# arkworks-rs/circom-compat

Measured on AMD Instinct MI355X. Metric: Groth16 constraints/sec (BN254), higher is better.
Workload: dtype int32x9 (29-bit limbs of 254-bit Montgomery integers); 1 GPU; synthetic squaring-chain R1CS, 2^22-2 constraints, BN254, full prove (witness map + 4 G1 MSM + 1 G2 MSM + finalize), trapdoor key minted on GPU; log2_domain=22, num_constraints=4194302, n_vars=4194304, parallelism=single-gpu

## Files before the change

### circom_compat_amd/csrc/api.hip

```cpp
#include "../../include/g16_amd.h"

#include <stddef.h>
#include <stdlib.h>

#include <algorithm>
#include <mutex>

#include "ctx.h"

using namespace g16;

static_assert(offsetof(g16::ProofSums, B1) == sizeof(g16::G1XYZZ29) && offsetof(g16::ProofSums, L) == 2 * sizeof(g16::G1XYZZ29),
              "ProofSums must keep A, B1, L adjacent (batched reduction writes them as an array)");
static_assert(G16_PARTIAL_BYTES == g16::FIN_PARTIAL_BYTES, "partial record size out of sync");

namespace {
std::mutex g_err_mu;
std::string g_create_error;
}


namespace {

g16_status fail(g16_ctx* ctx, g16_status code, const std::string& msg) {
  if (ctx) ctx->err = msg;
  else {
    std::lock_guard<std::mutex> g(g_err_mu);
    g_create_error = msg;
  }
  return code;
}

template <class Fn>
g16_status guarded(g16_ctx* ctx, Fn fn) {
  try {
    if (ctx) G16_HIP(hipSetDevice(ctx->device));
    return fn();
  } catch (const HipError& e) {
    return fail(ctx, G16_ERR_HIP, e.what());
  } catch (const std::bad_alloc&) {
    return fail(ctx, G16_ERR_INTERNAL, "host allocation failed");
  } catch (const std::exception& e) {
    const bool dom = std::string(e.what()).find("PolynomialDegreeTooLarge") != std::string::npos;
    return fail(ctx, dom ? G16_ERR_DOMAIN_TOO_LARGE : G16_ERR_INTERNAL, e.what());
  }
}

void shard(uint32_t len, int rank, int world, uint32_t* lo, uint32_t* hi) {
  *lo = (uint32_t)((uint64_t)len * rank / world);
  *hi = (uint32_t)((uint64_t)len * (rank + 1) / world);
}

int work1_batch(const MsmConfig& cw, uint32_t wr, bool sharded) {
  return (cw.nb() / wr < (1u << 18) || sharded) ? 3 : 2;
}

size_t msm_state_bytes(const MsmConfig& cw, const MsmConfig& ch, uint32_t lw, uint32_t l_cnt, uint32_t lh,
                       uint32_t wr, bool sharded, bool own_w, bool own_h, bool view_w) {
  size_t b = 0;
  if (view_w) b += MsmSort::view_bytes_for(lw, cw);
  if (own_w) b += (size_t)cw.Pn * ((size_t)lw * (64 * 2 + 128) + (size_t)l_cnt * 64);
  if (own_h) b += (size_t)ch.Pn * lh * 64;
  b += MsmSort::bytes_for(lw, cw) + MsmSort::bytes_for(lh, ch);
  const uint32_t nc_w = ceil_div(cw.B, msm_red_chunk(cw, 1, wr)) * cw.D;
  const uint32_t nc_h = ceil_div(ch.B, msm_red_chunk(ch)) * ch.D;
  const uint32_t slots_w = cw.nb() + cw.max_lanes(), slots_h = ch.nb() + ch.max_lanes();
  b += msm_work_bytes<Fq>(slots_w, nc_w, cw.D, work1_batch(cw, wr, sharded)) + msm_work_bytes<Fq2>(slots_w, nc_w, cw.D, 1) +
       msm_work_bytes<Fq>(slots_h, nc_h, ch.D, 1);
  return b;
}

void plan_msm_configs(const g16_options& o, uint32_t lw, uint32_t l_cnt, uint32_t lh, uint32_t wr, bool sharded,
                      bool own_w, bool own_h, bool view_w, MsmConfig* cw, MsmConfig* ch) {
  if (own_w) *cw = msm_make_config(lw ? lw : 1, o.window_bits, o.planes);
  if (own_h) *ch = msm_make_config(lh ? lh : 1, o.window_bits, o.planes);
  if (o.planes > 0) return;
  size_t fr = 0, tot = 0;
  if (hipMemGetInfo(&fr, &tot) != hipSuccess) return;
  const size_t margin = std::min(((size_t)2 << 30) + fr / 50, fr / 4);
  const size_t budget = fr - margin;
  if (msm_state_bytes(*cw, *ch, lw, l_cnt, lh, wr, sharded, own_w, own_h, view_w) <= budget) return;
  auto layouts = [&](const MsmConfig& full, uint32_t len, bool own) {
    std::vector<MsmConfig> v{full};
    for (int pn = full.Pn - 1; own && pn >= 1; --pn) {
      const MsmConfig c = msm_make_config(len ? len : 1, o.window_bits, pn);
      if (c.Pn != v.back().Pn) v.push_back(c);
    }
    return v;
  };
  const std::vector<MsmConfig> vw = layouts(*cw, lw, own_w), vh = layouts(*ch, lh, own_h);
  long best = -1;
  size_t best_bytes = 0;
  for (const MsmConfig& a : vw)
    for (const MsmConfig& b : vh) {
      const size_t need = msm_state_bytes(a, b, lw, l_cnt, lh, wr, sharded, own_w, own_h, view_w);
      if (need > budget) continue;
      const long score = 5L * a.D + b.D;
      if (best < 0 || score < best || (score == best && need > best_bytes)) {
        best = score;
        best_bytes = need;
        *cw = a;
        *ch = b;
      }
    }
  if (best < 0) {
    if (!own_w && !own_h)
      throw std::runtime_error("the sort and partial-sum state of this ctx does not fit the device memory that is free (" +
                               std::to_string(fr >> 20) + " MiB)");
    throw std::runtime_error("the proving key does not fit this device's memory even with one plane per point (" +
                             std::to_string(fr >> 20) + " MiB free)");
  }
}

inline bool sched_r5() {
  static const bool v = [] { const char* e = getenv("G16_SCHED_R5"); return e && atoi(e) != 0; }();
  return v;
}

void collect_times(g16_ctx* c) {
  if (c->timer.enabled) c->timer.collect(c->st_ms, c->st_cnt);
}

struct BucketChunk {
  uint32_t count;
  const Fr* w;
  size_t w_stride;
  int32_t *abc, *spmv;
  U256* h;
  ProofSums* sums;
  MsmSort *sort_w, *sort_h, *sort_b;
  MsmWork<Fq> *work1, *workH;
  MsmWork<Fq2>* work2;
  Fr* rs;
  const uint8_t* rs_host;
  FinScratch* scr;
  uint8_t *rec, *proj;
  uint32_t rec_stride;
  uint8_t *rec_host, *proj_host;
  const MsmSort& sort_for_b(const g16_ctx* c) const { return c->sparse_b ? *sort_b : *sort_w; }
};

BucketChunk own_chunk(g16_ctx* c, const Fr* w_dev) {
  return BucketChunk{1,           w_dev,       c->N,        c->wm.abc.p, c->wm.spmv.partial.p, c->h_canon.p, c->sums_dev.p,
                     &c->sort_w,  &c->sort_h,  &c->sort_b,  &c->work1,   &c->workH,            &c->work2,
                     c->rs_dev.p, c->pin_io,   c->fin_scr.p, c->out_dev.p, c->part_dev(), (uint32_t)G16_PROOF_BYTES,
                     c->pin_io + 64, c->pin_io + 64 + G16_PROOF_BYTES};
}

void accumulate_ab(g16_ctx* c, const BucketChunk& ch, hipStream_t s, StageTimer* tm, bool fixup = true) {
  if (c->ptsA.stride == 2) {
    msm_accumulate_pair<Fq>(*ch.sort_w, c->ptsA, c->ptsB1, *ch.work1, 0, s, tm, fixup);
  } else {
    msm_accumulate<Fq>(*ch.sort_w, c->ptsA, 0, *ch.work1, 0, s, tm, fixup);
    msm_accumulate<Fq>(*ch.sort_w, c->ptsB1, 0, *ch.work1, 1, s, tm, fixup);
  }
}
void fixup_ab(g16_ctx* c, const BucketChunk& ch, hipStream_t q) {
  StageTimer* tm = c->timer.enabled ? &c->timer : nullptr;
  if (c->ptsA.stride == 2) {
    msm_fixup_pair<Fq>(*ch.sort_w, c->ptsA, c->ptsB1, *ch.work1, 0, q, tm);
  } else {
    msm_fixup<Fq>(*ch.sort_w, c->ptsA, 0, *ch.work1, 0, q, tm);
    msm_fixup<Fq>(*ch.sort_w, c->ptsB1, 0, *ch.work1, 1, q, tm);
  }
}

void enqueue_witness_sort(g16_ctx* c, const BucketChunk& ch) {
  hipStream_t s = c->stream;
  StageTimer* tm = c->timer.enabled ? &c->timer : nullptr;
  int id = tm ? tm->begin(ST_MSM_SORT, s) : -1;
  ch.sort_w->run(ch.w + 1 + c->w_lo, c->w_hi - c->w_lo, true, s, ch.count, ch.w_stride);
  if (tm) tm->end(id, s);
  if (c->sparse_b) {
    hipStream_t v = c->overlap ? c->red : s;
    G16_HIP(hipEventRecord(c->ev_view, s));
    G16_HIP(hipStreamWaitEvent(v, c->ev_view, 0));
    id = tm ? tm->begin(ST_MSM_SORT, v) : -1;
    ch.sort_b->run_view(*ch.sort_w, c->keep_b, v);
    if (tm) tm->end(id, v);
    G16_HIP(hipEventRecord(c->ev_view, v));
  }
}
void wait_for_b_view(g16_ctx* c, hipStream_t s) {
  if (c->sparse_b) G16_HIP(hipStreamWaitEvent(s, c->ev_view, 0));
}

template <class Hook, class Hook2>
void enqueue_witness_msms(g16_ctx* c, const BucketChunk& ch, Hook after_ab, Hook2 after_b2, bool sorted = false) {
  hipStream_t s = c->stream;
  StageTimer* tm = c->timer.enabled ? &c->timer : nullptr;
  ProofSums* S = ch.sums;
  const size_t ps = sizeof(ProofSums);
  if (!sorted) enqueue_witness_sort(c, ch);
  const uint32_t nb_eff = ch.count * c->cfg_w.nb() / (c->shard_buckets ? (uint32_t)c->world : 1u);
  const bool small = nb_eff < (1u << 18);
  const uint32_t b2_limit = c->world > 1 ? (1u << 18) : (1u << 16);
  const bool b2_off = c->overlap && nb_eff < b2_limit;
  const bool sharded = c->world > 1 || c->dist_wm;
  const bool mid = (nb_eff >= (1u << 15) && small) || (sharded && nb_eff >= (1u << 15));
  if (mid && c->overlap && ch.work1->batch >= 3) {
    hipStream_t q = c->red;
    accumulate_ab(c, ch, s, tm, false);
    G16_HIP(hipEventRecord(c->ev_acc[0], s));
    G16_HIP(hipStreamWaitEvent(q, c->ev_acc[0], 0));
    fixup_ab(c, ch, q);
    msm_reduce<Fq>(*ch.sort_w, *ch.work1, 0, 2, &S->A, q, tm, true, ps);
    after_ab(q);
    wait_for_b_view(c, s);
    msm_accumulate<Fq2>(ch.sort_for_b(c), c->ptsB2, 0, *ch.work2, 0, s, tm);
    G16_HIP(hipEventRecord(c->ev_acc[1], s));
    G16_HIP(hipStreamWaitEvent(q, c->ev_acc[1], 0));
    msm_reduce<Fq2>(ch.sort_for_b(c), *ch.work2, 0, 1, &S->B2, q, tm, true, ps);
    const bool r5 = sched_r5();
    hipStream_t ql = r5 ? q : c->side;
    if (!r5) after_b2();
    msm_accumulate<Fq>(*ch.sort_w, c->ptsL, c->l_idx_min, *ch.work1, 2, s, tm, false);
    G16_HIP(hipEventRecord(c->ev_acc[2], s));
    G16_HIP(hipStreamWaitEvent(ql, c->ev_acc[2], 0));
    msm_fixup<Fq>(*ch.sort_w, c->ptsL, c->l_idx_min, *ch.work1, 2, ql, tm);
    msm_reduce<Fq>(*ch.sort_w, *ch.work1, 2, 1, &S->L, ql, tm, true, ps);
    if (r5) after_b2();
    G16_HIP(hipEventRecord(c->ev_b2, q));
    G16_HIP(hipStreamWaitEvent(c->side, c->ev_b2, 0));
    G16_HIP(hipEventRecord(c->ev_side, c->side));
    return;
  }
  if (small && ch.work1->batch >= 3) {
    accumulate_ab(c, ch, s, tm);
    msm_accumulate<Fq>(*ch.sort_w, c->ptsL, c->l_idx_min, *ch.work1, 2, s, tm);
    msm_reduce<Fq>(*ch.sort_w, *ch.work1, 0, 3, &S->A, s, tm, false, ps);
    after_ab(s);
  } else {
    accumulate_ab(c, ch, s, tm);
    msm_reduce<Fq>(*ch.sort_w, *ch.work1, 0, 2, &S->A, s, tm, false, ps);
    after_ab(s);
    msm_run<Fq>(*ch.sort_w, c->ptsL, c->l_idx_min, *ch.work1, &S->L, s, tm, ps);
  }
  wait_for_b_view(c, s);
  msm_accumulate<Fq2>(ch.sort_for_b(c), c->ptsB2, 0, *ch.work2, 0, s, tm);
  hipStream_t rs = b2_off ? c->red : s;
  G16_HIP(hipEventRecord(c->ev_b2, s));
  G16_HIP(hipStreamWaitEvent(rs, c->ev_b2, 0));
  msm_reduce<Fq2>(ch.sort_for_b(c), *ch.work2, 0, 1, &S->B2, rs, tm, false, ps);
  G16_HIP(hipEventRecord(c->ev_b2, rs));
  if (rs != c->red) G16_HIP(hipStreamWaitEvent(c->red, c->ev_b2, 0));
  after_b2();
  G16_HIP(hipEventRecord(c->ev_b2, c->red));
  G16_HIP(hipStreamWaitEvent(c->side, c->ev_b2, 0));
  G16_HIP(hipEventRecord(c->ev_side, c->side));
}

void enqueue_h_msm(g16_ctx* c, const BucketChunk& ch) {
  hipStream_t s = c->stream;
  StageTimer* tm = c->timer.enabled ? &c->timer : nullptr;
  G16_HIP(hipStreamWaitEvent(s, c->ev_h, 0));
  msm_run<Fq>(*ch.sort_h, c->ptsH, 0, *ch.workH, &ch.sums->H, s, tm, sizeof(ProofSums));
}

template <class Hook, class Hook2>
void run_msms(g16_ctx* c, const BucketChunk& ch, Hook after_ab, Hook2 after_b2) {
  hipStream_t s = c->stream, x = c->overlap ? c->aux : c->stream;
  StageTimer* tm = c->timer.enabled ? &c->timer : nullptr;
  const uint32_t nb_eff = ch.count * c->cfg_w.nb() / (c->shard_buckets ? (uint32_t)c->world : 1u);
  const bool sort_first = !sched_r5() && c->overlap && c->world == 1 && nb_eff >= (1u << 18) && c->n <= (1u << 24);
  if (sort_first) enqueue_witness_sort(c, ch);
  G16_HIP(hipEventRecord(c->ev_w, s));
  G16_HIP(hipStreamWaitEvent(x, c->ev_w, 0));
  int id = tm ? tm->begin(ST_WITNESS_MAP, x) : -1;
  c->wm.run_batch(ch.w, ch.w_stride, ch.count, ch.abc, ch.spmv, ch.h, nullptr, x);
  if (tm) tm->end(id, x);
  id = tm ? tm->begin(ST_MSM_SORT, x) : -1;
  ch.sort_h->run(ch.h + c->h_lo, c->h_hi - c->h_lo, false, x, ch.count, c->wm.n);
  if (tm) tm->end(id, x);
  G16_HIP(hipEventRecord(c->ev_h, x));
  enqueue_witness_msms(c, ch, after_ab, after_b2, sort_first);
  enqueue_h_msm(c, ch);
}

template <class Hook>
void run_msms(g16_ctx* c, const BucketChunk& ch, Hook after_ab) {
  run_msms(c, ch, after_ab, [] {});
}

void begin_sharded(g16_ctx* c, const uint64_t r[4], const uint64_t s_[4]) {
  hipStream_t s = c->stream;
  memcpy(c->fixed_rs, r, 32);
  memcpy(c->fixed_rs + 4, s_, 32);
  G16_HIP(hipMemcpyAsync(c->rs_dev.p, c->fixed_rs, 64, hipMemcpyHostToDevice, s));
  G16_HIP(hipEventRecord(c->ev_start, s));
  G16_HIP(hipStreamWaitEvent(c->side, c->ev_start, 0));
  fin_fixed_dist(c->fin_tab.p, c->rs_dev.p, c->fin_scr.p, c->side);
  c->fixed_ready = true;
}

g16_status check_w(g16_ctx* c, size_t n_vars) {
  if (n_vars != c->N) return fail(c, G16_ERR_INVALID, "witness length != n_vars of the key");
  return G16_OK;
}

}

namespace g16 {

void rank_collect_times(g16_ctx* c) { collect_times(c); }

struct TabChunk {
  uint32_t count;
  const Fr* w;
  uint32_t w_stride;
  Fr* rs;
  const uint8_t* rs_host;
  int32_t *abc, *spmv;
  U256* h;
  ProofSums* sums;
  FinScratch* scr;
  G1XYZZ29 *part1, *partH;
  G2XYZZ29* part2;
  uint8_t *proj, *proj_host;
};

static void enqueue_prove_tables(g16_ctx* c, const TabChunk& ch) {
  hipStream_t s = c->stream;
  hipStream_t x = c->overlap ? c->red : s, q = c->overlap ? c->aux : s, sd = c->overlap ? c->side : s;
  StageTimer* tm = c->timer.enabled ? &c->timer : nullptr;
  const uint32_t n = ch.count;
  G16_HIP(hipMemcpyAsync(ch.rs, ch.rs_host, (size_t)64 * n, hipMemcpyHostToDevice, s));
  G16_HIP(hipEventRecord(c->ev_start, s));
  G16_HIP(hipStreamWaitEvent(q, c->ev_start, 0));
  int id = tm ? tm->begin(ST_MSM_TABLE_G2, q) : -1;
  c->tbl.run_g2_witness(ch.w + 1, ch.w_stride, ch.sums, ch.part2, n, q);
  if (tm) tm->end(id, q);
  G16_HIP(hipStreamWaitEvent(x, c->ev_start, 0));
  id = tm ? tm->begin(ST_WITNESS_MAP, x) : -1;
  c->wm.run_batch(ch.w, ch.w_stride, n, ch.abc, ch.spmv, ch.h, nullptr, x);
  if (tm) tm->end(id, x);
  id = tm ? tm->begin(ST_MSM_TABLE_G1, x) : -1;
  c->tbl.run_h(ch.h, c->wm.n, ch.sums, ch.partH, n, x);
  if (tm) tm->end(id, x);
  G16_HIP(hipEventRecord(c->ev_h, x));
  G16_HIP(hipStreamWaitEvent(sd, c->ev_start, 0));
  fin_fixed_dist(c->fin_tab.p, ch.rs, ch.scr, sd, n);
  fin_tab_pre(c->key_dev.p, ch.scr, sd, n);
  G16_HIP(hipEventRecord(c->ev_fixed, sd));
  G16_HIP(hipStreamWaitEvent(q, c->ev_fixed, 0));
  fin_tab_b(ch.sums, ch.scr, ch.proj, q, n);
  G16_HIP(hipEventRecord(c->ev_b2, q));
  id = tm ? tm->begin(ST_MSM_TABLE_G1, s) : -1;
  c->tbl.run_g1_witness(ch.w + 1, ch.w_stride, ch.rs, ch.sums, ch.part1, n, s);
  if (tm) tm->end(id, s);
  G16_HIP(hipStreamWaitEvent(s, c->ev_fixed, 0));
  id = tm ? tm->begin(ST_FINALIZE, s) : -1;
  fin_tab_ac(ch.sums, ch.scr, ch.proj, s, n);
  G16_HIP(hipStreamWaitEvent(s, c->ev_h, 0));
  fin_tab_c(ch.sums, ch.scr, ch.proj, s, n);
  if (tm) tm->end(id, s);
  G16_HIP(hipStreamWaitEvent(s, c->ev_b2, 0));
  G16_HIP(hipMemcpyAsync(ch.proj_host, ch.proj, (size_t)FIN_PROJ_BYTES * n, hipMemcpyDeviceToHost, s));
}

static void enqueue_prove_tables(g16_ctx* c, const Fr* w_dev) {
  const TabChunk ch{1,           w_dev,          c->N,          c->rs_dev.p,   c->pin_io,
                    c->wm.abc.p, c->wm.spmv.partial.p, c->h_canon.p, c->sums_dev.p, c->fin_scr.p,
                    c->tbl.part1.p, c->tbl.partH.p, c->tbl.part2.p, c->part_dev(), c->pin_io + 64 + G16_PROOF_BYTES};
  enqueue_prove_tables(c, ch);
}

static void proof_from_pin(g16_ctx* c, uint8_t* proof_out) {
  if (c->tbl.active) {
    fin_tab_host_affine(c->pin_io + 64 + G16_PROOF_BYTES, proof_out);
  } else {
    memcpy(proof_out, c->pin_io + 64, G16_PROOF_BYTES);
    fin_host_affine_c(c->pin_io + 64 + G16_PROOF_BYTES, proof_out);
  }
}

static void enqueue_prove_buckets(g16_ctx* c, const BucketChunk& ch) {
  hipStream_t s = c->stream;
  const uint32_t n = ch.count;
  G16_HIP(hipMemcpyAsync(ch.rs, ch.rs_host, (size_t)64 * n, hipMemcpyHostToDevice, s));
  G16_HIP(hipEventRecord(c->ev_start, s));
  G16_HIP(hipStreamWaitEvent(c->side, c->ev_start, 0));
  fin_fixed(c->fin_tab.p, ch.rs, ch.scr, c->side, n);
  G16_HIP(hipEventRecord(c->ev_fixed, c->side));
  run_msms(
      c, ch,
      [&](hipStream_t from) {
        G16_HIP(hipEventRecord(c->ev_ab, from));
        G16_HIP(hipStreamWaitEvent(c->side, c->ev_ab, 0));
        fin_var(c->key_dev.p, ch.sums, ch.rs, ch.scr, ch.rec, c->side, n, ch.rec_stride);
// ... 1172 lines not shown
```

### circom_compat_amd/csrc/field29.h

```cpp
#pragma once
#include "field.h"

#if defined(G16_EMU) && !defined(F29_NO_CHECK)
#include <assert.h>
#include <math.h>
#define F29_CHECK 1
#endif

namespace g16 {

namespace f29 {

constexpr int N = 9;
constexpr uint32_t MASK = (1u << 29) - 1u;

G16_HD int32_t opaque(int32_t x) {
#if defined(__HIP_DEVICE_COMPILE__) && !defined(F29_NO_OPAQUE)
  asm("" : "+v"(x));
#endif
  return x;
}

#if defined(F29_CHAIN_MAD) && defined(__HIP_DEVICE_COMPILE__)
__device__ __forceinline__ void mad_vv(int64_t& acc, int32_t a, int32_t b) {
// ... 361 lines not shown
    for (int k = 0; k < 2 * f29::N - 1; ++k) {
      __int128 s = 0;
      for (int i = 0; i < f29::N; ++i) {
        const int j = k - i;
        if (j < 0 || j >= f29::N) continue;
        __int128 x = (__int128)a.l[i] * b.l[j];
        __int128 y = (__int128)c.l[i] * d.l[j];
        s += (x < 0 ? -x : x) + (y < 0 ? -y : y);
      }
      s += (__int128)9 << 58;
      s += (__int128)1 << 36;
      assert(s < ((__int128)1 << 63) && "F29 mul2: column overflow");
    }
    long double v = fabsl(approx_over_p(a) * approx_over_p(b)) + fabsl(approx_over_p(c) * approx_over_p(d));
    assert(v < 168.9L && "F29 mul2: value bound exceeded");
  }
  static void check_mul_inputs(const F29& a, const F29& b) {
    {
      long double v = fabsl(approx_over_p(a) * approx_over_p(b));
      assert(v < 168.9L && "F29 mul: value bound exceeded");
    }
    for (int k = 0; k < 2 * f29::N - 1; ++k) {
      __int128 s = 0;
      for (int i = 0; i < f29::N; ++i) {
        const int j = k - i;
        if (j < 0 || j >= f29::N) continue;
        __int128 x = (__int128)a.l[i] * b.l[j];
        s += x < 0 ? -x : x;
      }
      s += (__int128)9 << 58;
      s += (__int128)1 << 36;
      assert(s < ((__int128)1 << 63) && "F29 mul: column overflow");
    }
  }
#endif
};

template <class P>
G16_HD F29<P> f29_inv(const F29<P>& a) {
  uint32_t e[8];
#pragma unroll
  for (int i = 0; i < 8; ++i) e[i] = P::MOD[i];
  e[0] -= 2;
  F29<P> r = F29<P>::one();
  bool started = false;
  for (int i = 7; i >= 0; --i) {
    for (int bit = 31; bit >= 0; --bit) {
      if (started) r = r.sqr();
      if ((e[i] >> bit) & 1) {
        r = r * a;
        started = true;
      }
    }
  }
  return r;
}

template <class P>
G16_HD F29<P> f29_inv_vartime(const F29<P>& a) {
  uint32_t u[8], v[8], x1[8], x2[8];
  a.canonical().pack(u);
  uint32_t nz = 0;
#pragma unroll
  for (int i = 0; i < 8; ++i) {
    nz |= u[i];
    v[i] = P::MOD[i];
    x1[i] = 0;
    x2[i] = 0;
  }
  if (!nz) return F29<P>::zero();
  x1[0] = 1;
  auto is_one = [](const uint32_t* t) {
    uint32_t o = t[0] ^ 1u;
    for (int i = 1; i < 8; ++i) o |= t[i];
    return o == 0;
  };
  auto shr1 = [](uint32_t* t, uint32_t top) {
    for (int i = 0; i < 7; ++i) t[i] = (t[i] >> 1) | (t[i + 1] << 31);
    t[7] = (t[7] >> 1) | (top << 31);
  };
  auto halve_mod = [&](uint32_t* x) {
    uint32_t top = 0;
    if (x[0] & 1u) {
      uint64_t c = 0;
      for (int i = 0; i < 8; ++i) {
        c += (uint64_t)x[i] + P::MOD[i];
        x[i] = (uint32_t)c;
        c >>= 32;
      }
      top = (uint32_t)c;
    }
    shr1(x, top);
  };
  auto geq = [](const uint32_t* s, const uint32_t* t) {
    for (int i = 7; i >= 0; --i)
      if (s[i] != t[i]) return s[i] > t[i];
    return true;
  };
  auto sub = [](uint32_t* s, const uint32_t* t) {
    uint64_t br = 0;
    for (int i = 0; i < 8; ++i) {
      const uint64_t d = (uint64_t)s[i] - t[i] - br;
      s[i] = (uint32_t)d;
      br = (d >> 32) & 1;
    }
    return (uint32_t)br;
  };
  auto sub_mod = [&](uint32_t* s, const uint32_t* t) {
    if (sub(s, t)) {
      uint64_t c = 0;
      for (int i = 0; i < 8; ++i) {
        c += (uint64_t)s[i] + P::MOD[i];
        s[i] = (uint32_t)c;
        c >>= 32;
      }
    }
  };
  for (int guard = 0; guard < 2048 && !is_one(u) && !is_one(v); ++guard) {
    while (!(u[0] & 1u)) {
      shr1(u, 0);
      halve_mod(x1);
    }
    while (!(v[0] & 1u)) {
      shr1(v, 0);
      halve_mod(x2);
    }
    if (geq(u, v)) {
      sub(u, v);
      sub_mod(x1, x2);
    } else {
      sub(v, u);
      sub_mod(x2, x1);
    }
  }
  const uint32_t(&res)[8] = is_one(u) ? x1 : x2;
  return F29<P>::unpack(res) * F29<P>::from_limbs(F29<P>::C::R3);
}

template <class P>
struct F29x2 {
  F29<P> c0, c1;
  using B = F29<P>;
  static G16_HD F29x2 zero() { return F29x2{B::zero(), B::zero()}; }
  static G16_HD F29x2 one() { return F29x2{B::one(), B::zero()}; }
  G16_HD bool limbs_all_zero() const { return c0.limbs_all_zero() && c1.limbs_all_zero(); }
  friend G16_HD F29x2 operator+(const F29x2& a, const F29x2& b) { return F29x2{a.c0 + b.c0, a.c1 + b.c1}; }
  friend G16_HD F29x2 operator-(const F29x2& a, const F29x2& b) { return F29x2{a.c0 - b.c0, a.c1 - b.c1}; }
  G16_HD F29x2 neg() const { return F29x2{c0.neg(), c1.neg()}; }
  G16_HD F29x2 dbl() const { return F29x2{c0.dbl(), c1.dbl()}; }
  G16_HD F29x2 carry() const { return F29x2{c0.carry(), c1.carry()}; }
  friend G16_HD F29x2 operator*(const F29x2& a, const F29x2& b) {
    return F29x2{B::mul_sub(a.c0, b.c0, a.c1, b.c1), B::mul2(a.c0, b.c1, a.c1, b.c0)};
  }
  G16_HD F29x2 sqr() const { return F29x2{B::mul_sub(c0, c0, c1, c1), c0.dbl() * c1}; }
  static G16_HD F29x2 mul_sub(const F29x2& a, const F29x2& b, const F29x2& c, const F29x2& d) {
    return (a * b - c * d).carry();
  }
  G16_HD bool is_zero_mod_p() const { return c0.is_zero_mod_p() && c1.is_zero_mod_p(); }
  G16_HD bool maybe_zero_mod_p() const { return c0.maybe_zero_mod_p() && c1.maybe_zero_mod_p(); }
  G16_HD F29x2 canonical() const { return F29x2{c0.canonical(), c1.canonical()}; }
  static G16_HD F29x2 from_mont256(const Fq2& a) {
    return F29x2{B::from_mont256(a.c0), B::from_mont256(a.c1)};
  }
  G16_HD Fq2 to_mont256() const { return Fq2{c0.to_mont256(), c1.to_mont256()}; }
};
template <class P>
G16_HD F29x2<P> f29_inv(const F29x2<P>& a) {
  F29<P> n = f29_inv(F29<P>::mul2(a.c0, a.c0, a.c1, a.c1));
  return F29x2<P>{a.c0 * n, (a.c1 * n).neg()};
}
template <class P>
G16_HD F29x2<P> f29_inv_vartime(const F29x2<P>& a) {
  F29<P> n = f29_inv_vartime(F29<P>::mul2(a.c0, a.c0, a.c1, a.c1));
  return F29x2<P>{a.c0 * n, (a.c1 * n).neg()};
}

using Fq29 = F29<FqParams>;
using Fq2x29 = F29x2<FqParams>;

template <class F> struct Lazy;
template <> struct Lazy<Fq> {
  using type = F29<FqParams>;
  static G16_HD type load_packed(const Fq& raw) { return type::unpack(raw.v); }
  static G16_HD Fq store_packed(const type& a) {
    Fq r;
    a.pack_internal(r.v);
    return r;
  }
};
template <> struct Lazy<Fq2> {
  using type = F29x2<FqParams>;
  static G16_HD type load_packed(const Fq2& raw) {
    return type{F29<FqParams>::unpack_opaque(raw.c0.v), F29<FqParams>::unpack_opaque(raw.c1.v)};
  }
  static G16_HD Fq2 store_packed(const type& a) {
    Fq2 r;
    a.c0.pack_internal(r.c0.v);
    a.c1.pack_internal(r.c1.v);
    return r;
  }
};

using Fr29 = F29<FrParams>;

}
```

### circom_compat_amd/csrc/msm.h

```cpp
#pragma once
#include <stdlib.h>
#include "common.h"
#include "ec29.h"

namespace g16 {

constexpr int MSM_ACC_THREADS = 128;
#ifdef G16_EMU
constexpr int MSM_ACC_BLOCKS = 48;
constexpr int MSM_ACC_BLOCKS_G2 = 32;
#else
constexpr int MSM_ACC_BLOCKS = 3072;
constexpr int MSM_ACC_BLOCKS_G2 = 2048;
#endif
constexpr int MSM_MIN_SEG = 8;
constexpr int MSM_SMALL_MULTI = 32;
constexpr int MSM_RED_CHUNK = 16;
constexpr uint32_t MSM_IDX_BITS_WIDE = 27, MSM_IDX_BITS_NARROW = 26;

struct MsmConfig {
  int c = 0;
  int W = 0;
  int Pn = 1;
  int D = 0;
  uint32_t B = 0;
  uint32_t idx_bits = MSM_IDX_BITS_NARROW;
  uint32_t max_points() const { return 1u << idx_bits; }
  uint32_t lanes = MSM_ACC_BLOCKS * MSM_ACC_THREADS;
  uint32_t lanes2 = MSM_ACC_BLOCKS_G2 * MSM_ACC_THREADS;
  uint32_t nb() const { return (uint32_t)D * B; }
  uint32_t max_lanes() const { return lanes > lanes2 ? lanes : lanes2; }
};

constexpr int MSM_PART_BITS_MAX = 12;
inline int msm_part_bits(uint32_t nb) {
  int bits = 10;
  while (bits < MSM_PART_BITS_MAX && (((uint64_t)nb + ((uint64_t)1 << bits) - 1) >> bits) > 4096u) ++bits;
  return bits;
}
inline int msm_part_shift(uint32_t nb) {
  int bits = 0;
  while (((uint64_t)1 << bits) < nb) ++bits;
  const int pb = msm_part_bits(nb);
  return bits > pb ? bits - pb : 0;
}

inline uint32_t msm_red_chunk(const MsmConfig& cfg, uint32_t nbatch = 1, uint32_t world = 1, bool hidden = false) {
  const uint64_t per_launch = (uint64_t)nbatch * cfg.D * cfg.B / (world ? world : 1);
  const uint32_t target = (hidden && per_launch <= (1u << 17)) ? 32768u : 65536u;
  uint32_t ch = (uint32_t)(((uint64_t)nbatch * cfg.D * cfg.B) / ((uint64_t)target * (world ? world : 1)));
  if (ch < 1) ch = 1;
  if (ch > (uint32_t)MSM_RED_CHUNK) ch = (uint32_t)MSM_RED_CHUNK;
  if (world > 1) {
    uint32_t p2 = 1;
    while (p2 * 2 <= ch) p2 *= 2;
    ch = p2;
    const uint32_t part = 1u << msm_part_shift(cfg.nb());
    if (ch > part) ch = part;
  }
  return ch;
}

MsmConfig msm_make_config(size_t len, int c_override, int planes_override);

struct alignas(8) MsmPair {
  uint32_t x;
  uint32_t y;
};

G16_HD uint32_t msm_seg_len(uint32_t M, uint32_t lanes) {
  uint32_t S = (uint32_t)(((uint64_t)M + lanes - 1) / lanes);
  return S < (uint32_t)MSM_MIN_SEG ? (uint32_t)MSM_MIN_SEG : S;
}

struct MsmSort {
  MsmConfig cfg;
  uint32_t cap = 0, len = 0;
  uint32_t nproof = 1, nproof_cap = 1;
  uint32_t nbt() const { return nproof * cfg.nb(); }
  DevBuf<MsmPair> part;
  DevBuf<uint32_t> count, offset, cursor, entries, multi_l, meta, multi_l2, meta2, scan_tmp;
  uint32_t lanes_of(bool g2) const { return g2 ? cfg.lanes2 : cfg.lanes; }
  const uint32_t* large_list(bool g2) const { return g2 ? multi_l2.p : multi_l.p; }
  const uint32_t* large_meta(bool g2) const { return g2 ? meta2.p : meta.p; }
  DevBuf<uint32_t> part_off;
  DevBuf<uint32_t> blk_hist, blk_off;
  int rank = 0, world = 1;
  DevBuf<uint32_t> range;
  const uint32_t* range_dev() const { return world > 1 ? range.p : nullptr; }

  void init(uint32_t capacity, const MsmConfig& cfg, uint32_t nproof_cap = 1);
  void set_shard(int rank, int world);
  void run(const void* scalars, uint32_t n, bool mont, hipStream_t stream, uint32_t nproof = 1, size_t stride = 0);
  void init_view(uint32_t capacity, const MsmConfig& cfg, uint32_t nproof_cap = 1);
  void release_view() {
    count.release(); offset.release(); cursor.release(); entries.release(); multi_l.release();
    meta.release(); multi_l2.release(); meta2.release(); scan_tmp.release();
    cap = len = 0;
  }
  void run_view(const MsmSort& src, const uint32_t* keep_bits, hipStream_t stream);
  static size_t view_bytes_for(uint32_t capacity, const MsmConfig& cfg, uint32_t nproof = 1) {
    const uint64_t M = (uint64_t)nproof * capacity * cfg.W;
    return (size_t)(M * 4 + 3 * ((uint64_t)nproof * cfg.nb() + 1) * 4 + 2 * (M / ((uint64_t)MSM_MIN_SEG * MSM_SMALL_MULTI) + 2) * 4 + 4096);
  }
  size_t device_bytes() const;
  static size_t bytes_for(uint32_t capacity, const MsmConfig& cfg, uint32_t nproof = 1);
};

template <class F>
using MsmAcc = XYZZ29<typename Lazy<F>::type>;

template <class F>
struct MsmPoints {
  MsmConfig cfg;
  uint32_t count = 0;
  DevBuf<Affine<F>> pts;
  const Affine<F>* view = nullptr;
  uint32_t stride = 1, off = 0;
  const Affine<F>* data() const { return view ? view : pts.p; }
  void init(const Affine<F>* host_points, uint32_t count, const MsmConfig& cfg, hipStream_t stream);
  static void init_pair(MsmPoints& a, MsmPoints& b, const Affine<F>* host_a, const Affine<F>* host_b,
                        uint32_t count, const MsmConfig& cfg, hipStream_t stream);
  void init_from_device(const Affine<F>* dev_points, uint32_t count, const MsmConfig& cfg,
                        hipStream_t stream);
};

#ifdef G16_EMU
constexpr uint32_t MSM_FIX_CAP = 512;
#else
constexpr uint32_t MSM_FIX_CAP = 2048;
#endif
struct MsmFixList {
  uint32_t count;
  uint32_t overflow;
  uint32_t slot[MSM_FIX_CAP];
  uint32_t entry[MSM_FIX_CAP];
};

template <class F>
struct MsmWork {
  int batch = 1;
  uint32_t slots = 0, ncontrib = 0;
  int sets = 1;
  DevBuf<MsmAcc<F>> partial;
  DevBuf<MsmAcc<F>> contrib;
  DevBuf<MsmAcc<F>> bsum;
  DevBuf<MsmAcc<F>> wsum;
  DevBuf<MsmFixList> fix;
  void init(uint32_t n_slots, uint32_t n_contrib, int max_sets, int batch = 1);
};

template <class F>
inline size_t msm_work_bytes(uint32_t n_slots, uint32_t n_contrib, int max_sets, int batch) {
  return (size_t)batch * ((size_t)n_slots + n_contrib + (size_t)257 * max_sets) * sizeof(MsmAcc<F>) +
         (size_t)batch * sizeof(MsmFixList);
}

template <class F>
void msm_run(const MsmSort& s, const MsmPoints<F>& pts, uint32_t idx_min, MsmWork<F>& work,
             MsmAcc<F>* out_dev, hipStream_t stream, StageTimer* tm = nullptr, size_t out_stride = 0);
template <class F>
void msm_accumulate(const MsmSort& s, const MsmPoints<F>& pts, uint32_t idx_min, MsmWork<F>& work,
                    int slot, hipStream_t stream, StageTimer* tm = nullptr, bool fixup = true);
template <class F>
void msm_fixup(const MsmSort& s, const MsmPoints<F>& pts, uint32_t idx_min, MsmWork<F>& work, int slot,
               hipStream_t stream, StageTimer* tm = nullptr);
template <class F>
void msm_accumulate_pair(const MsmSort& s, const MsmPoints<F>& a, const MsmPoints<F>& b,
                         MsmWork<F>& work, int slot, hipStream_t stream, StageTimer* tm = nullptr,
                         bool fixup = true);
template <class F>
void msm_fixup_pair(const MsmSort& s, const MsmPoints<F>& a, const MsmPoints<F>& b, MsmWork<F>& work,
                    int slot, hipStream_t stream, StageTimer* tm = nullptr);
template <class F>
void msm_reduce(const MsmSort& s, MsmWork<F>& work, int first_slot, int nbatch, MsmAcc<F>* out_dev,
                hipStream_t stream, StageTimer* tm = nullptr, bool hidden = false, size_t out_stride = 0);
inline uint32_t msm_contrib_cap(const MsmConfig& cfg, uint32_t nproof_cap) {
  uint32_t m = 1;
  for (uint32_t z = 1; z <= nproof_cap; ++z)
    for (uint32_t nbatch = 1; nbatch <= 3; ++nbatch)
      for (int hidden = 0; hidden < 2; ++hidden) {
        const uint32_t rc = msm_red_chunk(cfg, nbatch * z, 1, hidden != 0);
        const uint32_t v = (uint32_t)(((uint64_t)cfg.B + rc - 1) / rc) * (uint32_t)cfg.D * z;
        if (v > m) m = v;
      }
  return m;
}



}
```

### circom_compat_amd/csrc/msm_curve.inc.h

```cpp
#pragma once
#include <stdlib.h>

#include "msm.h"

namespace g16 {

namespace {

constexpr int ACC_THREADS = MSM_ACC_THREADS;
constexpr uint32_t MSM_EXACT_BLOCKS = 256;

inline bool acc_fast() {
  static const bool v = [] { const char* e = getenv("G16_ACC_FAST"); return !e || atoi(e) != 0; }();
  return v;
}
template <class F>
constexpr bool acc_is_g1() { return sizeof(F) == sizeof(Fq); }
constexpr int COMB_THREADS = 64;
constexpr int SUM_THREADS = 128;

template <class F>
__global__ void __launch_bounds__(128) k_precompute_planes(Affine<F>* pts, uint32_t count, int Pn,
                                                           int shift_bits, uint32_t stride,
                                                           uint32_t off) {
// ... 424 lines not shown
  b.off = 1;
  a.pts.alloc((size_t)2 * c.Pn * (n ? n : 1));
  a.view = nullptr;
  b.view = a.pts.p;
  if (!n) return;
  const size_t rec = sizeof(Affine<F>);
  G16_HIP(hipMemcpy2DAsync(a.pts.p, 2 * rec, host_a, rec, rec, n, hipMemcpyHostToDevice, stream));
  G16_HIP(hipMemcpy2DAsync(a.pts.p + 1, 2 * rec, host_b, rec, rec, n, hipMemcpyHostToDevice, stream));
  for (uint32_t h = 0; h < 2; ++h)
    G16_LAUNCH((k_precompute_planes<F>), ceil_div(n, 128), 128, 0, stream, a.pts.p, n, c.Pn,
               c.c * c.D, 2u, h);
}

template <class F>
void MsmWork<F>::init(uint32_t n_slots, uint32_t n_contrib, int max_sets, int batch_) {
  slots = n_slots ? n_slots : 1;
  ncontrib = n_contrib ? n_contrib : 1;
  sets = max_sets;
  batch = batch_;
  partial.alloc((size_t)batch * slots);
  contrib.alloc((size_t)batch * ncontrib);
  bsum.alloc((size_t)batch * 256 * sets);
  wsum.alloc((size_t)batch * sets);
  fix.alloc((size_t)batch);
  G16_HIP(hipMemset(fix.p, 0, (size_t)batch * sizeof(MsmFixList)));
}

template <class F>
void msm_accumulate(const MsmSort& s, const MsmPoints<F>& P, uint32_t idx_min, MsmWork<F>& work,
                    int slot, hipStream_t stream, StageTimer* tm, bool fixup) {
  const MsmConfig& cfg = s.cfg;
  const uint32_t nb = s.nbt();
  const int acc_stage = sizeof(F) == sizeof(Fq) ? ST_MSM_ACC_G1 : ST_MSM_ACC_G2;
  if (slot < 0 || slot >= work.batch) throw std::runtime_error("msm_accumulate: bad workspace slot");
  const uint32_t lanes = s.lanes_of(sizeof(F) != sizeof(Fq));
  const uint32_t grid = lanes / ACC_THREADS;
#ifdef G16_DEBUG_GATHER
  static const bool mask_set = [] {
    if (const char* e = getenv("G16_DEBUG_GATHER_MASK")) {
      const uint32_t m = (uint32_t)strtoul(e, nullptr, 0);
      G16_HIP(hipMemcpyToSymbol(HIP_SYMBOL(g_gather_mask), &m, sizeof m));
    }
    return true;
  }();
  (void)mask_set;
#endif
  int id = tm ? tm->begin(acc_stage, stream) : -1;
  MsmAcc<F>* out = work.partial.p + (size_t)slot * work.slots;
  const uint32_t* en = (const uint32_t*)s.entries.p;
  const uint32_t* of = (const uint32_t*)s.offset.p;
  if constexpr (acc_is_g1<F>()) {
    if (acc_fast()) {
      MsmFixList* fix = work.fix.p + slot;
      if (P.stride == 2)
        G16_LAUNCH((k_bucket_accumulate<F, 2, false, true>), grid, ACC_THREADS, 0, stream, P.data() + P.off,
                   P.count, idx_min, cfg.idx_bits, en, of, nb, lanes, out, (size_t)0, fix);
      else
        G16_LAUNCH((k_bucket_accumulate<F, 1, false, true>), grid, ACC_THREADS, 0, stream, P.data(), P.count,
                   idx_min, cfg.idx_bits, en, of, nb, lanes, out, (size_t)0, fix);
      if (tm) tm->end(id, stream);
      if (fixup) msm_fixup<F>(s, P, idx_min, work, slot, stream, tm);
      return;
    }
  }
  if (P.stride == 2)
    G16_LAUNCH((k_bucket_accumulate<F, 2, false, false>), grid, ACC_THREADS, 0, stream, P.data() + P.off,
               P.count, idx_min, cfg.idx_bits, en, of, nb, lanes, out, (size_t)0, (MsmFixList*)nullptr);
  else
    G16_LAUNCH((k_bucket_accumulate<F, 1, false, false>), grid, ACC_THREADS, 0, stream, P.data(), P.count,
               idx_min, cfg.idx_bits, en, of, nb, lanes, out, (size_t)0, (MsmFixList*)nullptr);
  if (tm) tm->end(id, stream);
}

template <class F>
void msm_fixup(const MsmSort& s, const MsmPoints<F>& P, uint32_t idx_min, MsmWork<F>& work, int slot,
               hipStream_t stream, StageTimer* tm) {
  if constexpr (!acc_is_g1<F>()) {
    return;
  } else {
  if (!acc_fast()) return;
  const int tid = tm ? tm->begin(ST_MSM_FIXUP, stream) : -1;
  const MsmConfig& cfg = s.cfg;
  const uint32_t nb = s.nbt();
  const uint32_t lanes = s.lanes_of(sizeof(F) != sizeof(Fq));
  const uint32_t grid = lanes / ACC_THREADS;
  MsmAcc<F>* out = work.partial.p + (size_t)slot * work.slots;
  const uint32_t* en = (const uint32_t*)s.entries.p;
  const uint32_t* of = (const uint32_t*)s.offset.p;
  MsmFixList* fix = work.fix.p + slot;
  const uint32_t grid_x = grid < MSM_EXACT_BLOCKS ? grid : MSM_EXACT_BLOCKS;
  if (P.stride == 2) {
    G16_LAUNCH((k_acc_fixup<F, 2>), 1, 256, 0, stream, P.data() + P.off, P.count, idx_min, cfg.idx_bits, fix, out, (size_t)0);
    G16_LAUNCH((k_bucket_accumulate<F, 2, false, false>), grid_x, ACC_THREADS, 0, stream, P.data() + P.off,
               P.count, idx_min, cfg.idx_bits, en, of, nb, lanes, out, (size_t)0, fix);
  } else {
    G16_LAUNCH((k_acc_fixup<F, 1>), 1, 256, 0, stream, P.data(), P.count, idx_min, cfg.idx_bits, fix, out, (size_t)0);
    G16_LAUNCH((k_bucket_accumulate<F, 1, false, false>), grid_x, ACC_THREADS, 0, stream, P.data(), P.count,
               idx_min, cfg.idx_bits, en, of, nb, lanes, out, (size_t)0, fix);
  }
  if (tm) tm->end(tid, stream);
  }
}

template <class F>
void msm_accumulate_pair(const MsmSort& s, const MsmPoints<F>& A, const MsmPoints<F>& B,
                         MsmWork<F>& work, int slot, hipStream_t stream, StageTimer* tm, bool fixup) {
  const MsmConfig& cfg = s.cfg;
  const uint32_t nb = s.nbt();
  const int acc_stage = ST_MSM_ACC_G1_PAIR;
  if (slot < 0 || slot + 2 > work.batch) throw std::runtime_error("msm_accumulate_pair: bad workspace slot");
  if (A.stride != 2 || B.stride != 2 || A.data() != B.data() || A.off != 0 || B.off != 1 ||
      A.count != B.count)
    throw std::runtime_error("msm_accumulate_pair: the queries are not an interleaved pair");
  const uint32_t grid = cfg.lanes / (ACC_THREADS / 2);
  int id = tm ? tm->begin(acc_stage, stream) : -1;
  const uint32_t* en = (const uint32_t*)s.entries.p;
  const uint32_t* of = (const uint32_t*)s.offset.p;
  MsmAcc<F>* out = work.partial.p + (size_t)slot * work.slots;
  if constexpr (sizeof(F) == sizeof(Fq)) {
    if (acc_fast()) {
      G16_LAUNCH((k_bucket_accumulate<F, 2, true, true>), grid, ACC_THREADS, 0, stream, A.data(), A.count, 0u,
                 cfg.idx_bits, en, of, nb, cfg.lanes, out, (size_t)work.slots, work.fix.p + slot);
      if (tm) tm->end(id, stream);
      if (fixup) msm_fixup_pair<F>(s, A, B, work, slot, stream, tm);
      return;
    }
  }
  G16_LAUNCH((k_bucket_accumulate<F, 2, true, false>), grid, ACC_THREADS, 0, stream, A.data(), A.count, 0u,
             cfg.idx_bits, en, of, nb, cfg.lanes, out, (size_t)work.slots, (MsmFixList*)nullptr);
  if (tm) tm->end(id, stream);
}

template <class F>
void msm_fixup_pair(const MsmSort& s, const MsmPoints<F>& A, const MsmPoints<F>& B, MsmWork<F>& work,
                    int slot, hipStream_t stream, StageTimer* tm) {
  (void)B;
  if constexpr (sizeof(F) == sizeof(Fq)) {
    if (!acc_fast()) return;
    const int tid = tm ? tm->begin(ST_MSM_FIXUP, stream) : -1;
    const MsmConfig& cfg = s.cfg;
    const uint32_t nb = s.nbt();
    const uint32_t grid = cfg.lanes / (ACC_THREADS / 2);
    MsmAcc<F>* out = work.partial.p + (size_t)slot * work.slots;
    MsmFixList* fix = work.fix.p + slot;
    const uint32_t grid_x = grid < MSM_EXACT_BLOCKS ? grid : MSM_EXACT_BLOCKS;
    G16_LAUNCH((k_acc_fixup<F, 2>), 1, 256, 0, stream, A.data(), A.count, 0u, cfg.idx_bits, fix, out, (size_t)work.slots);
    G16_LAUNCH((k_bucket_accumulate<F, 2, true, false>), grid_x, ACC_THREADS, 0, stream, A.data(), A.count, 0u,
               cfg.idx_bits, (const uint32_t*)s.entries.p, (const uint32_t*)s.offset.p, nb, cfg.lanes, out,
               (size_t)work.slots, fix);
    if (tm) tm->end(tid, stream);
  }
}

template <class F>
void msm_reduce(const MsmSort& s, MsmWork<F>& work, int first_slot, int nbatch, MsmAcc<F>* out_dev,
                hipStream_t stream, StageTimer* tm, bool hidden, size_t out_stride) {
  const MsmConfig& cfg = s.cfg;
  const uint32_t nb = s.nbt();
  const uint32_t sets = (uint32_t)cfg.D * s.nproof;
  if (first_slot < 0 || nbatch < 1 || first_slot + nbatch > work.batch)
    throw std::runtime_error("msm_reduce: bad workspace slots");
  MsmAcc<F>* partial = work.partial.p + (size_t)first_slot * work.slots;
  int id = tm ? tm->begin(ST_MSM_REDUCE, stream) : -1;
  const bool g2 = sizeof(F) != sizeof(Fq);
  const uint32_t lanes = s.lanes_of(g2);
  G16_LAUNCH((k_combine_large<F>), dim3(1024, nbatch), COMB_THREADS, COMB_THREADS * sizeof(MsmAcc<F>),
             stream, s.large_list(g2), s.large_meta(g2),
             (const uint32_t*)s.offset.p, nb, lanes, partial, (size_t)work.slots);
  const uint32_t* rng = s.range_dev();
  const uint32_t red_chunk = msm_red_chunk(cfg, (uint32_t)nbatch * s.nproof, (uint32_t)s.world, hidden);
  const uint32_t cps = ceil_div(cfg.B, red_chunk);
  const uint32_t nchunks = cps * sets;
  if (nchunks > work.ncontrib) throw std::runtime_error("msm_reduce: contribution buffer too small");
  if ((int)sets > work.sets) throw std::runtime_error("msm_reduce: more bucket sets than the workspace holds");
  MsmAcc<F>* contrib = work.contrib.p + (size_t)first_slot * work.ncontrib;
  MsmAcc<F>* bsum = work.bsum.p + (size_t)first_slot * 256 * work.sets;
  MsmAcc<F>* wsum = work.wsum.p + (size_t)first_slot * work.sets;
  G16_LAUNCH((k_bucket_reduce<F>), dim3(ceil_div(nchunks, 64), nbatch), 64, 0, stream,
             (const MsmAcc<F>*)partial, (const uint32_t*)s.offset.p, nb, lanes, cfg.B, red_chunk,
             cps, nchunks, contrib, (size_t)work.slots, rng);
  uint32_t nblk = ceil_div(cps / (uint32_t)s.world, SUM_THREADS * 2);
  if (nblk > 256) nblk = 256;
  if (nblk < 1) nblk = 1;
  G16_LAUNCH((k_set_sum<F>), dim3(sets * nblk, nbatch), SUM_THREADS,
             SUM_THREADS * sizeof(MsmAcc<F>), stream, (const MsmAcc<F>*)contrib, cps, nblk,
             bsum, (size_t)nchunks, (size_t)256 * work.sets, rng, red_chunk);
  G16_LAUNCH((k_set_sum<F>), dim3(sets, nbatch), SUM_THREADS,
             SUM_THREADS * sizeof(MsmAcc<F>), stream, (const MsmAcc<F>*)bsum, nblk, 1u,
             wsum, (size_t)256 * work.sets, (size_t)work.sets, (const uint32_t*)nullptr, 1u);
  G16_LAUNCH((k_horner<F>), dim3(nbatch, s.nproof), 64, 0, stream, (const MsmAcc<F>*)wsum, work.sets, cfg.D,
             cfg.c, out_dev, out_stride);
  if (tm) tm->end(id, stream);
}

template <class F>
void msm_run(const MsmSort& s, const MsmPoints<F>& P, uint32_t idx_min, MsmWork<F>& work,
             MsmAcc<F>* out_dev, hipStream_t stream, StageTimer* tm, size_t out_stride) {
  msm_accumulate<F>(s, P, idx_min, work, 0, stream, tm);
  msm_reduce<F>(s, work, 0, 1, out_dev, stream, tm, false, out_stride);
}

}
```

### circom_compat_amd/csrc/msm_g1.hip

```cpp
#include "msm_curve.inc.h"
namespace g16 {
template struct MsmPoints<Fq>;
template struct MsmWork<Fq>;
template void msm_run<Fq>(const MsmSort&, const MsmPoints<Fq>&, uint32_t, MsmWork<Fq>&, MsmAcc<Fq>*,
                          hipStream_t, StageTimer*, size_t);
template void msm_accumulate<Fq>(const MsmSort&, const MsmPoints<Fq>&, uint32_t, MsmWork<Fq>&, int,
                                 hipStream_t, StageTimer*, bool);
template void msm_fixup<Fq>(const MsmSort&, const MsmPoints<Fq>&, uint32_t, MsmWork<Fq>&, int, hipStream_t, StageTimer*);
template void msm_accumulate_pair<Fq>(const MsmSort&, const MsmPoints<Fq>&, const MsmPoints<Fq>&,
                                      MsmWork<Fq>&, int, hipStream_t, StageTimer*, bool);
template void msm_fixup_pair<Fq>(const MsmSort&, const MsmPoints<Fq>&, const MsmPoints<Fq>&, MsmWork<Fq>&, int,
                                 hipStream_t, StageTimer*);
template void msm_reduce<Fq>(const MsmSort&, MsmWork<Fq>&, int, int, MsmAcc<Fq>*, hipStream_t,
                             StageTimer*, bool, size_t);
}
```

### circom_compat_amd/csrc/msm_g2.hip

```cpp
#include "msm_curve.inc.h"
namespace g16 {
template struct MsmPoints<Fq2>;
template struct MsmWork<Fq2>;
template void msm_run<Fq2>(const MsmSort&, const MsmPoints<Fq2>&, uint32_t, MsmWork<Fq2>&,
                           MsmAcc<Fq2>*, hipStream_t, StageTimer*, size_t);
template void msm_accumulate<Fq2>(const MsmSort&, const MsmPoints<Fq2>&, uint32_t, MsmWork<Fq2>&, int,
                                 hipStream_t, StageTimer*, bool);
template void msm_fixup<Fq2>(const MsmSort&, const MsmPoints<Fq2>&, uint32_t, MsmWork<Fq2>&, int, hipStream_t, StageTimer*);
template void msm_reduce<Fq2>(const MsmSort&, MsmWork<Fq2>&, int, int, MsmAcc<Fq2>*, hipStream_t,
                             StageTimer*, bool, size_t);
}
```

Baseline: 116.7 million constraints/s.

## Split MSM reduce into head/tail and overlap tails on side streams

Splits msm_reduce into a head (combine_large plus bucket_reduce) and a tail (set sums plus Horner). The tails of the A/B1, L and B2 reductions now run on the red or aux stream, so the main stream can start the next accumulate earlier. This is on by default (G16_TAIL_SPLIT=2) when overlap is enabled and the run is not sharded or small. Separately, Fq2 squaring now uses the (c0+c1)(c0-c1) form, replacing one dual-product mul_sub with a single multiply. The extra events and streams add sync overhead, and the tails compete with accumulate for compute units.

Result: faster. 118.5 million constraints/s, median of 6 (+1.5%).

```diff
diff --git a/circom_compat_amd/csrc/api.hip b/circom_compat_amd/csrc/api.hip
--- a/circom_compat_amd/csrc/api.hip
+++ b/circom_compat_amd/csrc/api.hip
@@ -115,6 +115,12 @@
 inline bool sched_r5() {
   static const bool v = [] { const char* e = getenv("G16_SCHED_R5"); return e && atoi(e) != 0; }();
   return v;
+}
+
+inline int tail_split(const g16_ctx* c, bool sharded) {
+  static const int v = [] { const char* e = getenv("G16_TAIL_SPLIT"); return e ? atoi(e) : 2; }();
+  if (!c->overlap || sharded || sched_r5()) return 0;
+  return v < 0 ? 0 : v > 3 ? 3 : v;
 }
 
 void collect_times(g16_ctx* c) {
@@ -231,10 +237,45 @@
     msm_reduce<Fq>(*ch.sort_w, *ch.work1, 0, 3, &S->A, s, tm, false, ps);
     after_ab(s);
   } else {
+    const int ts = small ? 0 : tail_split(c, sharded);
+    hipStream_t q = ts >= 1 ? c->red : s;
     accumulate_ab(c, ch, s, tm);
-    msm_reduce<Fq>(*ch.sort_w, *ch.work1, 0, 2, &S->A, s, tm, false, ps);
-    after_ab(s);
-    msm_run<Fq>(*ch.sort_w, c->ptsL, c->l_idx_min, *ch.work1, &S->L, s, tm, ps);
+    if (q == s) {
+      msm_reduce<Fq>(*ch.sort_w, *ch.work1, 0, 2, &S->A, s, tm, false, ps);
+      after_ab(s);
+      msm_run<Fq>(*ch.sort_w, c->ptsL, c->l_idx_min, *ch.work1, &S->L, s, tm, ps);
+    } else {
+      msm_reduce_head<Fq>(*ch.sort_w, *ch.work1, 0, 2, s, tm);
+      G16_HIP(hipEventRecord(c->ev_acc[0], s));
+      G16_HIP(hipStreamWaitEvent(q, c->ev_acc[0], 0));
+      msm_reduce_tail<Fq>(*ch.sort_w, *ch.work1, 0, 2, &S->A, q, tm, false, ps);
+      G16_HIP(hipEventRecord(c->ev_acc[1], q));
+      after_ab(q);
+      msm_accumulate<Fq>(*ch.sort_w, c->ptsL, c->l_idx_min, *ch.work1, 0, s, tm);
+      G16_HIP(hipStreamWaitEvent(s, c->ev_acc[1], 0));
+      msm_reduce_head<Fq>(*ch.sort_w, *ch.work1, 0, 1, s, tm);
+      G16_HIP(hipEventRecord(c->ev_acc[2], s));
+      G16_HIP(hipStreamWaitEvent(q, c->ev_acc[2], 0));
+      msm_reduce_tail<Fq>(*ch.sort_w, *ch.work1, 0, 1, &S->L, q, tm, false, ps);
+    }
+    if (ts >= 2) {
+      hipStream_t qb = ts == 3 ? c->aux : c->red;
+      wait_for_b_view(c, s);
+      msm_accumulate<Fq2>(ch.sort_for_b(c), c->ptsB2, 0, *ch.work2, 0, s, tm);
+      msm_reduce_head<Fq2>(ch.sort_for_b(c), *ch.work2, 0, 1, s, tm);
+      G16_HIP(hipEventRecord(c->ev_b2, s));
+      G16_HIP(hipStreamWaitEvent(qb, c->ev_b2, 0));
+      msm_reduce_tail<Fq2>(ch.sort_for_b(c), *ch.work2, 0, 1, &S->B2, qb, tm, false, ps);
+      if (qb != c->red) {
+        G16_HIP(hipEventRecord(c->ev_b2, qb));
+        G16_HIP(hipStreamWaitEvent(c->red, c->ev_b2, 0));
+      }
+      after_b2();
+      G16_HIP(hipEventRecord(c->ev_b2, c->red));
+      G16_HIP(hipStreamWaitEvent(c->side, c->ev_b2, 0));
+      G16_HIP(hipEventRecord(c->ev_side, c->side));
+      return;
+    }
   }
   wait_for_b_view(c, s);
   msm_accumulate<Fq2>(ch.sort_for_b(c), c->ptsB2, 0, *ch.work2, 0, s, tm);
diff --git a/circom_compat_amd/csrc/field29.h b/circom_compat_amd/csrc/field29.h
--- a/circom_compat_amd/csrc/field29.h
+++ b/circom_compat_amd/csrc/field29.h
@@ -537,7 +537,7 @@
   friend G16_HD F29x2 operator*(const F29x2& a, const F29x2& b) {
     return F29x2{B::mul_sub(a.c0, b.c0, a.c1, b.c1), B::mul2(a.c0, b.c1, a.c1, b.c0)};
   }
-  G16_HD F29x2 sqr() const { return F29x2{B::mul_sub(c0, c0, c1, c1), c0.dbl() * c1}; }
+  G16_HD F29x2 sqr() const { return F29x2{(c0 + c1).carry() * (c0 - c1), c0.dbl() * c1}; }
   static G16_HD F29x2 mul_sub(const F29x2& a, const F29x2& b, const F29x2& c, const F29x2& d) {
     return (a * b - c * d).carry();
   }
diff --git a/circom_compat_amd/csrc/msm.h b/circom_compat_amd/csrc/msm.h
--- a/circom_compat_amd/csrc/msm.h
+++ b/circom_compat_amd/csrc/msm.h
@@ -175,6 +175,12 @@
 template <class F>
 void msm_reduce(const MsmSort& s, MsmWork<F>& work, int first_slot, int nbatch, MsmAcc<F>* out_dev,
                 hipStream_t stream, StageTimer* tm = nullptr, bool hidden = false, size_t out_stride = 0);
+template <class F>
+void msm_reduce_head(const MsmSort& s, MsmWork<F>& work, int first_slot, int nbatch, hipStream_t stream,
+                     StageTimer* tm = nullptr, bool hidden = false);
+template <class F>
+void msm_reduce_tail(const MsmSort& s, MsmWork<F>& work, int first_slot, int nbatch, MsmAcc<F>* out_dev,
+                     hipStream_t stream, StageTimer* tm = nullptr, bool hidden = false, size_t out_stride = 0);
 inline uint32_t msm_contrib_cap(const MsmConfig& cfg, uint32_t nproof_cap) {
   uint32_t m = 1;
   for (uint32_t z = 1; z <= nproof_cap; ++z)
diff --git a/circom_compat_amd/csrc/msm_curve.inc.h b/circom_compat_amd/csrc/msm_curve.inc.h
--- a/circom_compat_amd/csrc/msm_curve.inc.h
+++ b/circom_compat_amd/csrc/msm_curve.inc.h
@@ -600,44 +600,76 @@
   }
 }
 
+namespace {
+template <class F>
+struct ReducePlan {
+  uint32_t nb, sets, lanes, red_chunk, cps, nchunks, nblk;
+  const uint32_t* rng;
+  MsmAcc<F>*partial, *contrib, *bsum, *wsum;
+};
+template <class F>
+ReducePlan<F> reduce_plan(const MsmSort& s, MsmWork<F>& work, int first_slot, int nbatch, bool hidden) {
+  const MsmConfig& cfg = s.cfg;
+  if (first_slot < 0 || nbatch < 1 || first_slot + nbatch > work.batch)
+    throw std::runtime_error("msm_reduce: bad workspace slots");
+  ReducePlan<F> p;
+  p.nb = s.nbt();
+  p.sets = (uint32_t)cfg.D * s.nproof;
+  p.lanes = s.lanes_of(sizeof(F) != sizeof(Fq));
+  p.rng = s.range_dev();
+  p.red_chunk = msm_red_chunk(cfg, (uint32_t)nbatch * s.nproof, (uint32_t)s.world, hidden);
+  p.cps = ceil_div(cfg.B, p.red_chunk);
+  p.nchunks = p.cps * p.sets;
+  if (p.nchunks > work.ncontrib) throw std::runtime_error("msm_reduce: contribution buffer too small");
+  if ((int)p.sets > work.sets) throw std::runtime_error("msm_reduce: more bucket sets than the workspace holds");
+  p.nblk = ceil_div(p.cps / (uint32_t)s.world, SUM_THREADS * 2);
+  if (p.nblk > 256) p.nblk = 256;
+  if (p.nblk < 1) p.nblk = 1;
+  p.partial = work.partial.p + (size_t)first_slot * work.slots;
+  p.contrib = work.contrib.p + (size_t)first_slot * work.ncontrib;
+  p.bsum = work.bsum.p + (size_t)first_slot * 256 * work.sets;
+  p.wsum = work.wsum.p + (size_t)first_slot * work.sets;
+  return p;
+}
+}
+
+template <class F>
+void msm_reduce_head(const MsmSort& s, MsmWork<F>& work, int first_slot, int nbatch, hipStream_t stream,
+                     StageTimer* tm, bool hidden) {
+  const ReducePlan<F> p = reduce_plan<F>(s, work, first_slot, nbatch, hidden);
+  const bool g2 = sizeof(F) != sizeof(Fq);
+  int id = tm ? tm->begin(ST_MSM_REDUCE, stream) : -1;
+  G16_LAUNCH((k_combine_large<F>), dim3(1024, nbatch), COMB_THREADS, COMB_THREADS * sizeof(MsmAcc<F>),
+             stream, s.large_list(g2), s.large_meta(g2),
+             (const uint32_t*)s.offset.p, p.nb, p.lanes, p.partial, (size_t)work.slots);
+  G16_LAUNCH((k_bucket_reduce<F>), dim3(ceil_div(p.nchunks, 64), nbatch), 64, 0, stream,
+             (const MsmAcc<F>*)p.partial, (const uint32_t*)s.offset.p, p.nb, p.lanes, s.cfg.B, p.red_chunk,
+             p.cps, p.nchunks, p.contrib, (size_t)work.slots, p.rng);
+  if (tm) tm->end(id, stream);
+}
+
+template <class F>
+void msm_reduce_tail(const MsmSort& s, MsmWork<F>& work, int first_slot, int nbatch, MsmAcc<F>* out_dev,
+                     hipStream_t stream, StageTimer* tm, bool hidden, size_t out_stride) {
+  const ReducePlan<F> p = reduce_plan<F>(s, work, first_slot, nbatch, hidden);
+  int id = tm ? tm->begin(ST_MSM_REDUCE, stream) : -1;
+  G16_LAUNCH((k_set_sum<F>), dim3(p.sets * p.nblk, nbatch), SUM_THREADS,
+             SUM_THREADS * sizeof(MsmAcc<F>), stream, (const MsmAcc<F>*)p.contrib, p.cps, p.nblk,
+             p.bsum, (size_t)p.nchunks, (size_t)256 * work.sets, p.rng, p.red_chunk);
+  G16_LAUNCH((k_set_sum<F>), dim3(p.sets, nbatch), SUM_THREADS,
+             SUM_THREADS * sizeof(MsmAcc<F>), stream, (const MsmAcc<F>*)p.bsum, p.nblk, 1u,
+             p.wsum, (size_t)256 * work.sets, (size_t)work.sets, (const uint32_t*)nullptr, 1u);
+  G16_LAUNCH((k_horner<F>), dim3(nbatch, s.nproof), 64, 0, stream, (const MsmAcc<F>*)p.wsum, work.sets, s.cfg.D,
+             s.cfg.c, out_dev, out_stride);
+  if (tm) tm->end(id, stream);
+}
+
 template <class F>
 void msm_reduce(const MsmSort& s, MsmWork<F>& work, int first_slot, int nbatch, MsmAcc<F>* out_dev,
                 hipStream_t stream, StageTimer* tm, bool hidden, size_t out_stride) {
-  const MsmConfig& cfg = s.cfg;
-  const uint32_t nb = s.nbt();
-  const uint32_t sets = (uint32_t)cfg.D * s.nproof;
-  if (first_slot < 0 || nbatch < 1 || first_slot + nbatch > work.batch)
-    throw std::runtime_error("msm_reduce: bad workspace slots");
-  MsmAcc<F>* partial = work.partial.p + (size_t)first_slot * work.slots;
   int id = tm ? tm->begin(ST_MSM_REDUCE, stream) : -1;
-  const bool g2 = sizeof(F) != sizeof(Fq);
-  const uint32_t lanes = s.lanes_of(g2);
-  G16_LAUNCH((k_combine_large<F>), dim3(1024, nbatch), COMB_THREADS, COMB_THREADS * sizeof(MsmAcc<F>),
-             stream, s.large_list(g2), s.large_meta(g2),
-             (const uint32_t*)s.offset.p, nb, lanes, partial, (size_t)work.slots);
-  const uint32_t* rng = s.range_dev();
-  const uint32_t red_chunk = msm_red_chunk(cfg, (uint32_t)nbatch * s.nproof, (uint32_t)s.world, hidden);
-  const uint32_t cps = ceil_div(cfg.B, red_chunk);
-  const uint32_t nchunks = cps * sets;
-  if (nchunks > work.ncontrib) throw std::runtime_error("msm_reduce: contribution buffer too small");
-  if ((int)sets > work.sets) throw std::runtime_error("msm_reduce: more bucket sets than the workspace holds");
-  MsmAcc<F>* contrib = work.contrib.p + (size_t)first_slot * work.ncontrib;
-  MsmAcc<F>* bsum = work.bsum.p + (size_t)first_slot * 256 * work.sets;
-  MsmAcc<F>* wsum = work.wsum.p + (size_t)first_slot * work.sets;
-  G16_LAUNCH((k_bucket_reduce<F>), dim3(ceil_div(nchunks, 64), nbatch), 64, 0, stream,
-             (const MsmAcc<F>*)partial, (const uint32_t*)s.offset.p, nb, lanes, cfg.B, red_chunk,
-             cps, nchunks, contrib, (size_t)work.slots, rng);
-  uint32_t nblk = ceil_div(cps / (uint32_t)s.world, SUM_THREADS * 2);
-  if (nblk > 256) nblk = 256;
-  if (nblk < 1) nblk = 1;
-  G16_LAUNCH((k_set_sum<F>), dim3(sets * nblk, nbatch), SUM_THREADS,
-             SUM_THREADS * sizeof(MsmAcc<F>), stream, (const MsmAcc<F>*)contrib, cps, nblk,
-             bsum, (size_t)nchunks, (size_t)256 * work.sets, rng, red_chunk);
-  G16_LAUNCH((k_set_sum<F>), dim3(sets, nbatch), SUM_THREADS,
-             SUM_THREADS * sizeof(MsmAcc<F>), stream, (const MsmAcc<F>*)bsum, nblk, 1u,
-             wsum, (size_t)256 * work.sets, (size_t)work.sets, (const uint32_t*)nullptr, 1u);
-  G16_LAUNCH((k_horner<F>), dim3(nbatch, s.nproof), 64, 0, stream, (const MsmAcc<F>*)wsum, work.sets, cfg.D,
-             cfg.c, out_dev, out_stride);
+  msm_reduce_head<F>(s, work, first_slot, nbatch, stream, nullptr, hidden);
+  msm_reduce_tail<F>(s, work, first_slot, nbatch, out_dev, stream, nullptr, hidden, out_stride);
   if (tm) tm->end(id, stream);
 }
 
diff --git a/circom_compat_amd/csrc/msm_g1.hip b/circom_compat_amd/csrc/msm_g1.hip
--- a/circom_compat_amd/csrc/msm_g1.hip
+++ b/circom_compat_amd/csrc/msm_g1.hip
@@ -13,4 +13,7 @@
                                  hipStream_t, StageTimer*);
 template void msm_reduce<Fq>(const MsmSort&, MsmWork<Fq>&, int, int, MsmAcc<Fq>*, hipStream_t,
                              StageTimer*, bool, size_t);
+template void msm_reduce_head<Fq>(const MsmSort&, MsmWork<Fq>&, int, int, hipStream_t, StageTimer*, bool);
+template void msm_reduce_tail<Fq>(const MsmSort&, MsmWork<Fq>&, int, int, MsmAcc<Fq>*, hipStream_t,
+                                  StageTimer*, bool, size_t);
 }
diff --git a/circom_compat_amd/csrc/msm_g2.hip b/circom_compat_amd/csrc/msm_g2.hip
--- a/circom_compat_amd/csrc/msm_g2.hip
+++ b/circom_compat_amd/csrc/msm_g2.hip
@@ -9,4 +9,7 @@
 template void msm_fixup<Fq2>(const MsmSort&, const MsmPoints<Fq2>&, uint32_t, MsmWork<Fq2>&, int, hipStream_t, StageTimer*);
 template void msm_reduce<Fq2>(const MsmSort&, MsmWork<Fq2>&, int, int, MsmAcc<Fq2>*, hipStream_t,
                              StageTimer*, bool, size_t);
+template void msm_reduce_head<Fq2>(const MsmSort&, MsmWork<Fq2>&, int, int, hipStream_t, StageTimer*, bool);
+template void msm_reduce_tail<Fq2>(const MsmSort&, MsmWork<Fq2>&, int, int, MsmAcc<Fq2>*, hipStream_t,
+                                  StageTimer*, bool, size_t);
 }
```
